# hebbarashwin/neural_polar_decoder

Hardware: AMD Instinct MI355X
Metric: codewords/sec Polar(64,32) SC + CRISP-GRU decode, 1/2/4/8 GPU; BER match (higher is better)
Workload: dtype fp16x3 GRU (hi+lo fp16 MFMA operands, fp32 accumulate/gates); fp32 SC

## Files before the change

neural_polar_decoder_amd/csrc/npd_gru.hip:

```cpp
#include <stdlib.h>
#include <string.h>

#include <new>
#include <type_traits>
#include <vector>

#include "npd_common.hpp"
#include "npd_gru_common.hpp"

namespace npd {
namespace gru {

template <int F, int L, int WPB = NPD_GRU_WPB, int HDT = 0>
__global__ __launch_bounds__(64 * WPB) void gru_decode_kernel(const Args a) {
    constexpr bool FOLD = true, BINIT = true;
    using G = Geo<F, L>;
    constexpr int TT = G::TT, HT = G::HT, KG = G::KG;
    extern __shared__ __attribute__((aligned(16))) f4 smem4[];
    const float* smem = reinterpret_cast<const float*>(smem4);
    {
        const f4* src = reinterpret_cast<const f4*>(a.img);
        for (int i = threadIdx.x; i < G::TOTAL / 4; i += blockDim.x) smem4[i] = src[i];
        __syncthreads();
    }
    const int lane = threadIdx.x & 63;
    const int wave = threadIdx.x >> 6;
    const int half = lane >> 5;
    const int col = lane & 31;
    const int N = a.N;
    const int64_t ntiles = (a.B + 31) / 32;
    const f16v zero = {0.f, 0.f, 0.f, 0.f, 0.f, 0.f, 0.f, 0.f, 0.f, 0.f, 0.f, 0.f, 0.f, 0.f, 0.f, 0.f};
    auto cvec = [&](int off) -> f16v {
        const f4* p = reinterpret_cast<const f4*>(smem + off + half * 16);
        const f4 x0 = p[0], x1 = p[1], x2 = p[2], x3 = p[3];
        return f16v{x0[0], x0[1], x0[2], x0[3], x1[0], x1[1], x1[2], x1[3],
                    x2[0], x2[1], x2[2], x2[3], x3[0], x3[1], x3[2], x3[3]};
    };

    for (int64_t tile = (int64_t)blockIdx.x * WPB + wave; tile < ntiles; tile += (int64_t)gridDim.x * WPB) {
        const int64_t cw = tile * 32 + col;
        const bool valid = cw < a.B;
        const int64_t cwc = valid ? cw : a.B - 1;

        f16v P[TT];
#pragma unroll
        for (int t = 0; t < TT; ++t) P[t] = zero;
        if (a.y) {
            const f4* yr = reinterpret_cast<const f4*>(a.y + cwc * N + half * (N / 2));
            const int ng = N / 8;
            for (int s4 = 0; s4 < ng; ++s4) {
                const f4 yv = yr[s4];
#pragma unroll
                for (int t = 0; t < TT; ++t) {
                    const f4 w = a.wy[(t * ng + s4) * 64 + lane];
                    P[t] = mfma(w.x, yv.x, P[t]);
                    P[t] = mfma(w.y, yv.y, P[t]);
                    P[t] = mfma(w.z, yv.z, P[t]);
// ... 494 lines not shown
    const int64_t tiles = (a.B + 31) / 32;
    const int64_t wgs = (tiles + NPD_GRU_WPB - 1) / NPD_GRU_WPB;
    hipLaunchKernelGGL(kern, dim3(grid_for(wgs, 1, device_cu_count())), dim3(64 * NPD_GRU_WPB), lds, s, a);
    return launch_check("lstm_decode_kernel launch");
}

typedef __bf16 bf8 __attribute__((ext_vector_type(8)));
typedef _Float16 hf8 __attribute__((ext_vector_type(8)));

template <int SPLIT>
struct SplitT {
    static constexpr bool kLo = SPLIT >= 3;
    static constexpr bool kF16 = SPLIT >= 4;
    static constexpr bool kFold = SPLIT == 5;
    using V = std::conditional_t<kF16, hf8, bf8>;
    using E = std::conditional_t<kF16, _Float16, __bf16>;
    static constexpr float kIn = SPLIT == 4 ? 256.0f : 1.0f;
    static constexpr float kAcc = SPLIT == 4 ? 1.0f / 65536.0f : 1.0f;
    static constexpr float kC1 = kFold ? 1.0f : -1.44269504088896340736f * kAcc;
    static constexpr float kC2 = kFold ? 1.0f : -2.88539008177792681472f * kAcc;
};

template <int F, int L, int SPLIT>
struct GeoB {
    static constexpr int TT = 3 * F / 32, HT = F / 32, KB = F / 16;
    static constexpr int NG = (L == 2) ? 3 : 1;
    static constexpr int IMG = NG * TT * KB * 64 * 4;
    static constexpr int NS = SPLIT >= 3 ? 2 : 1;
    static constexpr int OFF_X = NS * IMG;
    static constexpr int OFF_IN = OFF_X + NG * TT * 64;
    static constexpr int OFF_WL = OFF_IN + HT * 64;
    static constexpr int TOTAL = OFF_WL + 2 * HT * 16;
};

struct ArgsB {
    const float* img;
    const f4* wy;
    const float* y;
    const float* h0;
    const float* gt;
    float* decoded;
    float* logits;
    int64_t B;
    int N;
    int rev;
    int onehot;
    float b_lin;
    int64_t wy_lo;
    uint32_t info[kMaxWords];
    const float* msg;
    unsigned long long* counters;
    int K;
    int nseg;
    uint32_t slotw[kMaxN / 4];
};

__device__ __forceinline__ f16v mfma16(const bf8& a, const bf8& b, const f16v& c) {
    return __builtin_amdgcn_mfma_f32_32x32x16_bf16(a, b, c, 0, 0, 0);
}
__device__ __forceinline__ f16v mfma16(const hf8& a, const hf8& b, const f16v& c) {
    return __builtin_amdgcn_mfma_f32_32x32x16_f16(a, b, c, 0, 0, 0);
}


template <int SPLIT>
__device__ __forceinline__ void gru_update_fast(f16v& h, const f16v& ar, const f16v& az, const f16v& ain,
                                                const f16v& ahn) {
    constexpr float c1 = SplitT<SPLIT>::kC1, c2 = SplitT<SPLIT>::kC2;
#pragma unroll
    for (int i = 0; i < 16; ++i) {
        const float r = __builtin_amdgcn_rcpf(1.0f + __builtin_amdgcn_exp2f(c1 * ar[i]));
        const float z = __builtin_amdgcn_rcpf(1.0f + __builtin_amdgcn_exp2f(c1 * az[i]));
        const float x = ain[i] + ahn[i] * r;
        const float nn = fmaf(2.0f, __builtin_amdgcn_rcpf(1.0f + __builtin_amdgcn_exp2f(c2 * x)), -1.0f);
        h[i] = (h[i] - nn) * z + nn;
    }
}

template <int HT, int SPLIT>
__device__ __forceinline__ void to_frags(const f16v (&h)[HT], typename SplitT<SPLIT>::V (&hi)[2 * HT],
                                         typename SplitT<SPLIT>::V (&lo)[2 * HT]) {
    using S = SplitT<SPLIT>;
#pragma unroll
    for (int t = 0; t < HT; ++t)
#pragma unroll
        for (int s = 0; s < 2; ++s)
#pragma unroll
            for (int j = 0; j < 8; ++j) {
                const float v = h[t][8 * s + j] * S::kIn;
                const typename S::E b = (typename S::E)v;
                hi[2 * t + s][j] = b;
                if (S::kLo) lo[2 * t + s][j] = (typename S::E)(v - (float)b);
            }
}

template <int TT, int KB, int NT, int SPLIT, int IMG>
__device__ __forceinline__ void gemm_bf(const f4* __restrict__ smem4, int g, int t0, int lane, f16v (&acc)[NT],
                                        const typename SplitT<SPLIT>::V (&hi)[KB],
                                        const typename SplitT<SPLIT>::V (&lo)[KB]) {
    using V = typename SplitT<SPLIT>::V;
#pragma unroll
    for (int q = 0; q < KB; ++q) {
        V ah[NT], al[NT];
#pragma unroll
        for (int t = 0; t < NT; ++t) {
            const f4 v = smem4[((g * TT + t0 + t) * KB + q) * 64 + lane];
            ah[t] = __builtin_bit_cast(V, v);
// ... 212 lines not shown
                        const size_t e = ((((size_t)(g * TT + t) * KB + q) * 64 + l) * 8 + j);
                        u16[e] = hi;
                        if (SPLIT >= 3) u16[(size_t)GB::IMG * 2 + e] = lo;
                    }
    const float kc = SPLIT == 4 ? 65536.0f : 1.0f;
    for (int i = 0; i < GB::NG * TT * 64; ++i) img[GB::OFF_X + i] = img32[G32::OFF_X + i] * kc;
    for (int i = 0; i < HT * 64; ++i) img[GB::OFF_IN + i] = img32[G32::OFF_IN + i] * kc;
    for (int i = 0; i < 2 * HT * 16; ++i) img[GB::OFF_WL + i] = img32[G32::OFF_WL + i];
    const int nq = N / 16;
    const size_t per = (size_t)TT * nq * 64 * 8;
    wy.assign((per * (SPLIT >= 3 ? 2 : 1) + 1) / 2, 0.0f);
    uint16_t* w16 = reinterpret_cast<uint16_t*>(wy.data());
    for (int t = 0; t < TT; ++t)
        for (int q = 0; q < nq; ++q)
            for (int l = 0; l < 64; ++l)
                for (int j = 0; j < 8; ++j) {
                    const int row = 32 * t + (l & 31);
                    const int k = 16 * q + 8 * (l >> 5) + j;
                    const float v = wih[0][(size_t)row * Din + k];
                    const size_t e = (((size_t)t * nq + q) * 64 + l) * 8 + j;
                    uint16_t hi, lo;
                    split16<SPLIT>(v, hi, lo);
                    w16[e] = hi;
                    if (SPLIT >= 3) w16[per + e] = lo;
                }
    wy_lo = (int64_t)(per / 8);
}

template <int F, int L, int SPLIT>
static int launch_bf(const npd_gru* g, const ArgsB& a, hipStream_t s) {
    using G = GeoB<F, L, SPLIT>;
    auto kern = gru_decode_bf_kernel<F, L, SPLIT>;
    const size_t lds = (size_t)G::TOTAL * 4;
    static bool attr = false;
    if (!attr) {
        NPD_HIP(hipFuncSetAttribute((const void*)kern, hipFuncAttributeMaxDynamicSharedMemorySize, 163840));
        attr = true;
    }
    const int64_t tiles = (a.B + 31) / 32;
    const int64_t wgs = (tiles + NPD_GRU_BF_WPB - 1) / NPD_GRU_BF_WPB;
    const int grid = grid_for(wgs, 1, device_cu_count());
    hipLaunchKernelGGL(kern, dim3(grid), dim3(64 * NPD_GRU_BF_WPB), lds, s, a);
    (void)g;
    return launch_check("gru_decode_bf_kernel launch");
}

struct Geo16 {
    static constexpr int RT = 12, KB = 2, NG = 3;
    static constexpr int IMG4 = NG * RT * KB * 64;
    static constexpr int G_BYTES = RT * KB * 2 * 1024;
    static constexpr int OFF_C = 2 * IMG4 * 4;
    static constexpr int C0L0 = OFF_C, C1L0 = OFF_C + 192, BHN0 = OFF_C + 384, C0L1 = OFF_C + 448,
                         BHN1 = OFF_C + 640, WLIN = OFF_C + 704, TOTAL = OFF_C + 768;
};

__device__ __forceinline__ f4 mfma16s(const hf8& a, const hf8& b, const f4& c) {
    return __builtin_amdgcn_mfma_f32_16x16x32_f16(a, b, c, 0, 0, 0);
}
__device__ __forceinline__ f4 mfma16s(const bf8& a, const bf8& b, const f4& c) {
    return __builtin_amdgcn_mfma_f32_16x16x32_bf16(a, b, c, 0, 0, 0);
}

template <int SPLIT>
__device__ __forceinline__ void split16s(const f4 (&h)[4], typename SplitT<SPLIT>::V (&hi)[2],
                                         typename SplitT<SPLIT>::V (&lo)[2]) {
    using S = SplitT<SPLIT>;
#pragma unroll
    for (int kb = 0; kb < 2; ++kb)
#pragma unroll
        for (int j = 0; j < 8; ++j) {
            const float v = h[2 * kb + (j >> 2)][j & 3] * S::kIn;
            const typename S::E b = (typename S::E)v;
            hi[kb][j] = b;
            if (S::kLo) lo[kb][j] = (typename S::E)(v - (float)b);
        }
}

__device__ __forceinline__ f4 frag16(const f4* __restrict__ smem4, uint32_t wb, int t, int kb, int part) {
    return *reinterpret_cast<const f4*>(reinterpret_cast<const char*>(smem4) + wb +
                                        ((t * Geo16::KB + kb) * 2 + part) * 1024);
}

__device__ __forceinline__ float sum_rows16(float p) {
    const auto r = __builtin_amdgcn_permlane16_swap(__float_as_uint(p), __float_as_uint(p), false, false);
    const float s = __uint_as_float(r[0]) + __uint_as_float(r[1]);
    const auto r2 = __builtin_amdgcn_permlane32_swap(__float_as_uint(s), __float_as_uint(s), false, false);
    return __uint_as_float(r2[0]) + __uint_as_float(r2[1]);
}

__device__ __forceinline__ f4 fma4(float x, const f4& c, const f4& p) {
    return f4{fmaf(x, c[0], p[0]), fmaf(x, c[1], p[1]), fmaf(x, c[2], p[2]), fmaf(x, c[3], p[3])};
}

#define NPD_GRU16_WPB 8
template <int SPLIT>
struct Upd4 {
    f4 er, ez, en, z;
    template <int C>
    __device__ __forceinline__ void step(f4& h, const f4& ar, const f4& az, const f4& ain, const f4& ahn) {
        constexpr float c1 = SplitT<SPLIT>::kC1, c2 = SplitT<SPLIT>::kC2;
        constexpr int i = C / 3, st = C % 3;
        if constexpr (st == 0) {
            er[i] = __builtin_amdgcn_exp2f(c1 * ar[i]);
            ez[i] = __builtin_amdgcn_exp2f(c1 * az[i]);
        } else if constexpr (st == 1) {
            const float r = __builtin_amdgcn_rcpf(1.0f + er[i]);
            z[i] = __builtin_amdgcn_rcpf(1.0f + ez[i]);
            en[i] = __builtin_amdgcn_exp2f(c2 * (ain[i] + ahn[i] * r));
        } else {
            const float nn = fmaf(2.0f, __builtin_amdgcn_rcpf(1.0f + en[i]), -1.0f);
            h[i] = (h[i] - nn) * z[i] + nn;
        }
    }
};

template <int SPLIT>
__device__ __forceinline__ void split_kb(const f4 (&h)[4], int kb, typename SplitT<SPLIT>::V (&hi)[2],
                                         typename SplitT<SPLIT>::V (&lo)[2]) {
    using S = SplitT<SPLIT>;
#pragma unroll
    for (int j = 0; j < 8; ++j) {
        const float v = h[2 * kb + (j >> 2)][j & 3] * S::kIn;
        const typename S::E b = (typename S::E)v;
        hi[kb][j] = b;
        if (S::kLo) lo[kb][j] = (typename S::E)(v - (float)b);
    }
}


template <int SPLIT, int NU>
struct Frag16 {
    typename SplitT<SPLIT>::V h[NU], l[NU];
};
template <int SPLIT, int NU>
__device__ __forceinline__ void load_kb16(const f4* __restrict__ smem4, uint32_t wb, const int (&t)[NU], int kb,
                                          Frag16<SPLIT, NU>& f) {
    using V = typename SplitT<SPLIT>::V;
#pragma unroll
    for (int u = 0; u < NU; ++u) {
        f.h[u] = __builtin_bit_cast(V, frag16(smem4, wb, t[u], kb, 0));
        if (SplitT<SPLIT>::kLo) f.l[u] = __builtin_bit_cast(V, frag16(smem4, wb, t[u], kb, 1));
    }
}

template <int SPLIT, int NU, int C0, int NCH, typename Work>
__device__ __forceinline__ void gemm16i(const f4* __restrict__ smem4, uint32_t wb, const int (&t)[NU],
                                        f4 (&acc)[NU], const typename SplitT<SPLIT>::V (&bh)[2],
                                        const typename SplitT<SPLIT>::V (&bl)[2], Frag16<SPLIT, NU>& cur,
                                        uint32_t wbn, const int (&tn)[NU], Work&& work) {
    constexpr int NT = 2 * NU;
    Frag16<SPLIT, NU> f[2];
    load_kb16<SPLIT, NU>(smem4, wb, t, 1, f[1]);
    asm volatile("" ::: "memory");
    static_for<0, NT>([&](auto trc) {
        constexpr int tr = decltype(trc)::value;
        constexpr int kb = tr / NU, u = tr % NU;
        const Frag16<SPLIT, NU>& F = kb == 0 ? cur : f[kb];
        acc[u] = mfma16s(F.h[u], bh[kb], acc[u]);
        if (SplitT<SPLIT>::kLo) {
            acc[u] = mfma16s(F.h[u], bl[kb], acc[u]);
            acc[u] = mfma16s(F.l[u], bh[kb], acc[u]);
        }
        if constexpr (tr == NU - 1) {
            asm volatile("" ::: "memory");
            load_kb16<SPLIT, NU>(smem4, wbn, tn, 0, cur);
        }
        static_for<C0 + NCH * tr / NT, C0 + NCH * (tr + 1) / NT>([&](auto cc) { work(cc); });
        __builtin_amdgcn_sched_barrier(0);
    });
}

template <int SPLIT>
__global__ __launch_bounds__(64 * NPD_GRU16_WPB) void gru16p_kernel(const ArgsB a) {
    using G = Geo16;
    using S = SplitT<SPLIT>;
    using V = typename S::V;
    using E = typename S::E;
    extern __shared__ __attribute__((aligned(16))) f4 smem4[];
    {
        const f4* src = reinterpret_cast<const f4*>(a.img);
        for (int i = threadIdx.x; i < G::TOTAL / 4; i += blockDim.x) smem4[i] = src[i];
        __syncthreads();
    }
    const int lane = threadIdx.x & 63;
    const int wave = threadIdx.x >> 6;
    const int g4 = lane >> 4;
    const int col = lane & 15;
    const int N = a.N;
    const int nkb = N / 32;
    const int64_t tps = (a.B + 15) / 16;
    const int64_t ntiles = tps * (a.nseg > 1 ? a.nseg : 1);
    const bool count = a.counters != nullptr;
    uint32_t be_w = 0, bl_w = 0;
    uint32_t wbs[3];
#pragma unroll
    for (int g = 0; g < 3; ++g) {
        uint32_t v = g * G::G_BYTES + lane * 16;
        asm volatile("" : "+v"(v));
        wbs[g] = v;
    }
    uint32_t cb = (G::OFF_C + 4 * g4) * 4;
    asm volatile("" : "+v"(cb));
    auto c4 = [&](int off, int t) -> f4 {
        return *reinterpret_cast<const f4*>(reinterpret_cast<const char*>(smem4) + cb + (off - G::OFF_C + 16 * t) * 4);
    };
    const f4 zero = {0.f, 0.f, 0.f, 0.f};
    constexpr int T0[3] = {0, 4, 8};
    auto nowork = [](auto) {};

    for (int64_t tile = (int64_t)blockIdx.x * NPD_GRU16_WPB + wave; tile < ntiles;
         tile += (int64_t)gridDim.x * NPD_GRU16_WPB) {
        const int64_t seg = tile / tps;
        const int64_t cw = (tile - seg * tps) * 16 + col;
        const bool valid = cw < a.B;
        const int64_t cwc = valid ? cw : a.B - 1;
        const int64_t rowoff = (seg * a.B + cw) * N;
        uint32_t mc[4] = {0u, 0u, 0u, 0u};
        if (count) {
            const float* mr = a.msg + cwc * a.K;
#pragma unroll
            for (int w = 0; w < 4; ++w)
                for (int j = 0; j < 16; ++j) {
                    const int sl = 4 * (16 * w + j) + g4;
                    if (sl >= a.K) break;
                    const float v = rintf(mr[sl]);
                    const uint32_t code = v == -1.0f ? 0u : v == 1.0f ? 1u : v == 0.0f ? 2u : 3u;
                    mc[w] |= code << (2 * j);
                }
        }
        uint32_t nerr = 0;
        f4 P[G::RT];
#pragma unroll
        for (int t = 0; t < G::RT; ++t) P[t] = c4(G::C0L0, t);
        if (a.y) {
            const float* yr = a.y + (seg * a.B + cwc) * N;
            for (int kb = 0; kb < nkb; ++kb) {
                const f4 y0 = *reinterpret_cast<const f4*>(yr + 32 * kb + 8 * g4);
                const f4 y1 = *reinterpret_cast<const f4*>(yr + 32 * kb + 8 * g4 + 4);
                V yh, yl;
#pragma unroll
                for (int j = 0; j < 8; ++j) {
                    const float v = (j < 4 ? y0[j] : y1[j - 4]) * S::kIn;
                    yh[j] = (E)v;
                    if (S::kLo) yl[j] = (E)(v - (float)yh[j]);
                }
#pragma unroll
                for (int t = 0; t < G::RT; ++t) {
                    const V wh = __builtin_bit_cast(V, a.wy[(t * nkb + kb) * 64 + lane]);
                    P[t] = mfma16s(wh, yh, P[t]);
                    if (S::kLo) {
                        const V wl = __builtin_bit_cast(V, a.wy[a.wy_lo + (t * nkb + kb) * 64 + lane]);
                        P[t] = mfma16s(wh, yl, P[t]);
                        P[t] = mfma16s(wl, yh, P[t]);
                    }
                }
            }
        }
        f4 h0[4], h1[4];
#pragma unroll
        for (int t = 0; t < 4; ++t) {
            h0[t] = zero;
            h1[t] = zero;
        }
        if (a.h0) {
            const float* hr = a.h0 + (seg * a.B + cwc) * 128;
#pragma unroll
            for (int t = 0; t < 4; ++t)
#pragma unroll
                for (int e = 0; e < 4; ++e) {
                    const int f = 16 * t + 4 * g4 + e;
                    h0[t][e] = hr[2 * f];
                    h1[t][e] = hr[2 * f + 1];
                }
        }
        V fh[2], fl[2], gh[2], gl[2];
        split16s<SPLIT>(h0, fh, fl);
        split16s<SPLIT>(h1, gh, gl);
        float xb = 1.0f;
        f4 a0[3] = {zero, zero, c4(G::BHN0, 0)};
        constexpr int T1[3] = {1, 5, 9};
        Frag16<SPLIT, 3> cur;
        load_kb16<SPLIT, 3>(smem4, wbs[0], T0, 0, cur);
        gemm16i<SPLIT, 3, 0, 0>(smem4, wbs[0], T0, a0, fh, fl, cur, wbs[0], T1, nowork);
        for (int ii = 0; ii < N; ++ii) {
            const int jj = a.rev ? N - 1 - ii : ii;
            Upd4<SPLIT> u;
            const int sl = count ? (int)((a.slotw[jj >> 2] >> (8 * (jj & 3))) & 255u) : 255;
            f4 ap[3] = {a0[0] + fma4(xb, c4(G::C1L0, 0), P[0]), a0[1] + fma4(xb, c4(G::C1L0, 4), P[4]), a0[2]};
            f4 ainp = fma4(xb, c4(G::C1L0, 8), P[8]);
            static_for<1, 4>([&](auto htc) {
                constexpr int ht = decltype(htc)::value;
                const int T[3] = {ht, 4 + ht, 8 + ht};
                f4 acc[3] = {fma4(xb, c4(G::C1L0, ht), P[ht]), fma4(xb, c4(G::C1L0, 4 + ht), P[4 + ht]),
                             c4(G::BHN0, ht)};
                constexpr int TN[3] = {ht < 3 ? ht + 1 : 0, ht < 3 ? 5 + ht : 4, ht < 3 ? 9 + ht : 8};
                gemm16i<SPLIT, 3, 0, 12>(smem4, wbs[0], T, acc, fh, fl, cur, wbs[ht < 3 ? 0 : 2], TN, [&](auto cc) {
                    u.template step<decltype(cc)::value>(h0[ht - 1], ap[0], ap[1], ainp, ap[2]);
                });
                ainp = fma4(xb, c4(G::C1L0, 8 + ht), P[8 + ht]);
#pragma unroll
                for (int k = 0; k < 3; ++k) ap[k] = acc[k];
            });
            f4 b[3] = {c4(G::C0L1, 0), c4(G::C0L1, 4), c4(G::BHN1, 0)};
            gemm16i<SPLIT, 3, 0, 14>(smem4, wbs[2], T0, b, gh, gl, cur, wbs[1], T0, [&](auto cc) {
                constexpr int c = decltype(cc)::value;
                if constexpr (c < 12) u.template step<c>(h0[3], ap[0], ap[1], ainp, ap[2]);
                else split_kb<SPLIT>(h0, c - 12, fh, fl);
            });
            f4 bi[3] = {b[0], b[1], c4(G::C0L1, 8)};
            gemm16i<SPLIT, 3, 0, 0>(smem4, wbs[1], T0, bi, fh, fl, cur, wbs[2], T1, nowork);
            f4 q[4] = {bi[0], bi[1], bi[2], b[2]};
            float part = 0.0f;
            static_for<1, 4>([&](auto htc) {
                constexpr int ht = decltype(htc)::value;
                const int T[3] = {ht, 4 + ht, 8 + ht};
                f4 bb[3] = {c4(G::C0L1, ht), c4(G::C0L1, 4 + ht), c4(G::BHN1, ht)};
                auto work = [&](auto cc) {
                    constexpr int c = decltype(cc)::value;
                    if constexpr (c < 12) {
                        u.template step<c>(h1[ht - 1], q[0], q[1], q[2], q[3]);
                    } else {
                        const f4 wl = c4(G::WLIN, ht - 1);
#pragma unroll
                        for (int i = 0; i < 4; ++i) part = fmaf(wl[i], h1[ht - 1][i], part);
                    }
                };
                gemm16i<SPLIT, 3, 0, 7>(smem4, wbs[2], T, bb, gh, gl, cur, wbs[1], T, work);
                f4 bbi[3] = {bb[0], bb[1], c4(G::C0L1, 8 + ht)};
                constexpr int TN[3] = {ht < 3 ? ht + 1 : 0, ht < 3 ? 5 + ht : 4, ht < 3 ? 9 + ht : 8};
                gemm16i<SPLIT, 3, 7, 6>(smem4, wbs[1], T, bbi, fh, fl, cur, wbs[ht < 3 ? 2 : 0], TN, work);
                q[0] = bbi[0];
                q[1] = bbi[1];
                q[2] = bbi[2];
                q[3] = bb[2];
            });
            a0[0] = zero;
            a0[1] = zero;
            a0[2] = c4(G::BHN0, 0);
            gemm16i<SPLIT, 3, 0, 15>(smem4, wbs[0], T0, a0, fh, fl, cur, wbs[0], T1, [&](auto cc) {
                constexpr int c = decltype(cc)::value;
                if constexpr (c < 12) {
                    u.template step<c>(h1[3], q[0], q[1], q[2], q[3]);
                } else if constexpr (c == 12) {
                    const f4 wl = c4(G::WLIN, 3);
#pragma unroll
                    for (int i = 0; i < 4; ++i) part = fmaf(wl[i], h1[3][i], part);
                    const float out = sum_rows16(part) + a.b_lin;
                    const bool info = (a.info[jj >> 5] >> (jj & 31)) & 1u;
                    float d;
                    if (info) d = out > 0.0f ? 1.0f : (out < 0.0f ? -1.0f : 0.0f);
                    else d = a.gt ? a.gt[(seg * a.B + cwc) * N + jj] : 1.0f;
                    if (g4 == 0 && valid) {
                        if (a.decoded) a.decoded[rowoff + jj] = d;
                        if (a.logits) a.logits[rowoff + ii] = out;
                    }
                    if (sl != 255) {
                        const int q = sl >> 2, w = q >> 4;
                        const uint32_t mw = w == 0 ? mc[0] : w == 1 ? mc[1] : w == 2 ? mc[2] : mc[3];
                        const uint32_t dc = d > 0.0f ? 1u : (d < 0.0f ? 0u : 2u);
                        nerr += (g4 == (sl & 3) && ((mw >> (2 * (q & 15))) & 3u) != dc) ? 1u : 0u;
                    }
                    const float sd = d > 0.0f ? 1.0f : (d < 0.0f ? -1.0f : 0.0f);
                    xb = a.onehot ? (sd > 0.0f ? 1.0f : 0.0f) : sd;
                } else {
                    split_kb<SPLIT>(h1, c - 13, gh, gl);
                }
            });
        }
        if (count) {
            nerr += __shfl_xor(nerr, 16, 64);
            nerr += __shfl_xor(nerr, 32, 64);
            const bool mine = g4 == 0 && valid;
            bl_w += (uint32_t)__builtin_popcountll(__ballot(mine && nerr != 0u));
            uint32_t e = mine ? nerr : 0u;
#pragma unroll
            for (int o = 1; o < 16; o <<= 1) e += __shfl_xor(e, o, 64);
            be_w += (uint32_t)__builtin_amdgcn_readfirstlane(e);
            const int64_t nt = tile + (int64_t)gridDim.x * NPD_GRU16_WPB;
            if (nt >= ntiles || nt / tps != seg) {
                if (lane == 0 && (be_w | bl_w)) {
                    atomicAdd(a.counters + 2 * seg, (unsigned long long)be_w);
                    atomicAdd(a.counters + 2 * seg + 1, (unsigned long long)bl_w);
                }
                be_w = bl_w = 0;
            }
        }
    }
}

template <int SPLIT>
static void build_image16(const float* W, int N, int onehot, std::vector<float>& img, std::vector<float>& wy,
                          int64_t& wy_lo) {
    using G = Geo16;
    constexpr int F = 64, L = 2;
    const int Din = N + (onehot ? 2 : 1);
    const float* p = W;
    const float* wih[2];
    const float* whh[2];
    const float* bih[2];
    const float* bhh[2];
    for (int l = 0; l < L; ++l) {
        const int din = l == 0 ? Din : F;
        wih[l] = p; p += (size_t)3 * F * din;
        whh[l] = p; p += (size_t)3 * F * F;
        bih[l] = p; p += 3 * F;
        bhh[l] = p; p += 3 * F;
    }
    const float* wlin = p;
    img.assign(G::TOTAL, 0.0f);
    const float* mats[3] = {whh[0], wih[1], whh[1]};
    auto fold = [&](int row) { return SPLIT == 5 ? (row < 2 * F ? -1.44269504088896340736f : -2.88539008177792681472f) : 1.0f; };
    uint16_t* u16 = reinterpret_cast<uint16_t*>(img.data());
    for (int g = 0; g < G::NG; ++g)
        for (int t = 0; t < G::RT; ++t)
            for (int kb = 0; kb < G::KB; ++kb)
                for (int l = 0; l < 64; ++l)
                    for (int j = 0; j < 8; ++j) {
                        const int row = 16 * t + (l & 15);
                        const int hid = 16 * (2 * kb + (j >> 2)) + 4 * (l >> 4) + (j & 3);
                        uint16_t hi, lo;
                        split16<SPLIT>(fold(row) * mats[g][(size_t)row * F + hid], hi, lo);
                        const size_t e = (((((size_t)(g * G::RT + t) * G::KB + kb) * 2) * 64 + l) * 8 + j);
                        u16[e] = hi;
                        if (SPLIT >= 3) u16[e + 64 * 8] = lo;
                    }
    const float kc = SPLIT == 4 ? 65536.0f : 1.0f;
    auto col = [&](int row, int k) { return wih[0][(size_t)row * Din + k]; };
    for (int row = 0; row < 3 * F; ++row) {
        const bool rz = row < 2 * F;
        const float c0x = onehot ? col(row, N) : 0.0f;
        const float c1x = onehot ? col(row, N + 1) - col(row, N) : col(row, N);
        img[G::C0L0 + row] = fold(row) * (kc * (rz ? bih[0][row] + bhh[0][row] + c0x : bih[0][row] + c0x));
        img[G::C1L0 + row] = fold(row) * (kc * c1x);
        img[G::C0L1 + row] = fold(row) * (kc * (rz ? bih[1][row] + bhh[1][row] : bih[1][row]));
    }
    for (int j = 0; j < F; ++j) {
        img[G::BHN0 + j] = fold(2 * F + j) * (kc * bhh[0][2 * F + j]);
        img[G::BHN1 + j] = fold(2 * F + j) * (kc * bhh[1][2 * F + j]);
        img[G::WLIN + j] = wlin[j];
    }
    const int nkb = N / 32;
    const size_t per = (size_t)G::RT * nkb * 64 * 8;
    wy.assign((per * (SPLIT >= 3 ? 2 : 1) + 1) / 2, 0.0f);
    uint16_t* w16 = reinterpret_cast<uint16_t*>(wy.data());
    for (int t = 0; t < G::RT; ++t)
        for (int kb = 0; kb < nkb; ++kb)
            for (int l = 0; l < 64; ++l)
                for (int j = 0; j < 8; ++j) {
                    const int row = 16 * t + (l & 15);
                    const int k = 32 * kb + 8 * (l >> 4) + j;
                    uint16_t hi, lo;
                    split16<SPLIT>(fold(row) * col(row, k), hi, lo);
                    const size_t e = (((size_t)t * nkb + kb) * 64 + l) * 8 + j;
                    w16[e] = hi;
                    if (SPLIT >= 3) w16[per + e] = lo;
                }
    wy_lo = (int64_t)(per / 8);
}

template <int SPLIT>
static int launch16(const ArgsB& a, hipStream_t s) {
    auto kern = gru16p_kernel<SPLIT>;
    static bool attr = false;
    if (!attr) {
        NPD_HIP(hipFuncSetAttribute((const void*)kern, hipFuncAttributeMaxDynamicSharedMemorySize, 163840));
        attr = true;
    }
    const int64_t tiles = (a.B + 15) / 16 * (a.nseg > 1 ? a.nseg : 1);
    const int64_t wgs = (tiles + NPD_GRU16_WPB - 1) / NPD_GRU16_WPB;
    const int grid = grid_for(wgs, 1, device_cu_count());
    hipLaunchKernelGGL(kern, dim3(grid), dim3(64 * NPD_GRU16_WPB), (size_t)Geo16::TOTAL * 4, s, a);
    return launch_check("gru16p_kernel launch");
}

template <int F>
struct WideGeo {
    static constexpr int HT = F / 32;
    static constexpr int NW = HT < 8 ? HT : 8;
    static constexpr int HPW = HT / NW;
};

int wide_lds_bytes(int N, int F, int L) {
    const int nw = (F / 32) < 8 ? F / 32 : 8;
    return (L * F * 32 + N * 32 + nw * 32) * 4;
}

template <int HPW, int D0, int D1, int D2>
__device__ __forceinline__ void wide_chain(const f4* __restrict__ W, int kg, int HT, int jt0,
                                           const f4* __restrict__ Bs, int lane, f16v (&acc)[4][HPW]) {
    constexpr int D[3] = {D0, D1, D2};
    f4 wc[3][HPW];
#pragma unroll
    for (int k = 0; k < 3; ++k)
#pragma unroll
        for (int j = 0; j < HPW; ++j) wc[k][j] = W[((size_t)(k * HT + jt0 + j) * kg + 0) * 64 + lane];
    for (int q = 0; q < kg; ++q) {
        f4 wn[3][HPW];
        if (q + 1 < kg) {
#pragma unroll
            for (int k = 0; k < 3; ++k)
#pragma unroll
                for (int j = 0; j < HPW; ++j) wn[k][j] = W[((size_t)(k * HT + jt0 + j) * kg + q + 1) * 64 + lane];
        }
        const f4 b = Bs[q * 64 + lane];
        asm volatile("" ::: "memory");
#pragma unroll
        for (int e = 0; e < 4; ++e)
#pragma unroll
            for (int k = 0; k < 3; ++k)
#pragma unroll
                for (int j = 0; j < HPW; ++j) acc[D[k]][j] = mfma(wc[k][j][e], b[e], acc[D[k]][j]);
        if (q + 1 < kg) {
#pragma unroll
            for (int k = 0; k < 3; ++k)
#pragma unroll
                for (int j = 0; j < HPW; ++j) wc[k][j] = wn[k][j];
        }
    }
}

template <int HPW>
__device__ __forceinline__ void wide_update(f4* __restrict__ Hs, int jt, int lane, f16v& hv, const f16v& ar,
                                            const f16v& az, const f16v& ain, const f16v& ahn) {
#pragma unroll
    for (int q = 0; q < 4; ++q) {
// ... 601 lines not shown
        b.wy = reinterpret_cast<const gru::f4*>(g->wy);
        b.y = y; b.h0 = h0; b.gt = gt; b.decoded = decoded; b.logits = logits; b.B = B; b.N = g->N;
        b.rev = a.rev; b.onehot = a.onehot; b.b_lin = g->b_lin; b.wy_lo = g->wy_lo;
        b.nseg = 1;
        for (int w = 0; w < kMaxWords; ++w) b.info[w] = a.info[w];
        if (g->img16) {
            b.img = g->img16;
            b.wy = reinterpret_cast<const gru::f4*>(g->wy16);
            b.wy_lo = g->wy16_lo;
            return g->split16 == 3 ? gru::launch16<3>(b, s) : g->split16 == 5 ? gru::launch16<5>(b, s)
                                   : gru::launch16<1>(b, s);
        }
#define NPD_LBF(FF, LL)                                                                                   \
        return g->precision == 1   ? gru::launch_bf<FF, LL, 3>(g, b, s)                                     \
               : g->precision == 3 ? gru::launch_bf<FF, LL, 4>(g, b, s)                                     \
                                   : gru::launch_bf<FF, LL, 1>(g, b, s)
        if (g->F == 64 && g->layers == 2) NPD_LBF(64, 2);
        if (g->F == 64) NPD_LBF(64, 1);
        if (g->layers == 2) NPD_LBF(32, 2);
        NPD_LBF(32, 1);
#undef NPD_LBF
    }
    if (g->F > 64) {
        if (g->F == 512) return g->layers == 2 ? gru::launch_wide<512, 2>(a, g->N, s) : gru::launch_wide<512, 1>(a, g->N, s);
        if (g->F == 256) return g->layers == 2 ? gru::launch_wide<256, 2>(a, g->N, s) : gru::launch_wide<256, 1>(a, g->N, s);
        return g->layers == 2 ? gru::launch_wide<128, 2>(a, g->N, s) : gru::launch_wide<128, 1>(a, g->N, s);
    }
    if (g->hd != nullptr) {
#define NPD_LHD(FF, LL) \
        return g->hd_tiles == 1 ? gru::launch<FF, LL, 1>(a, s) : g->hd_tiles == 2 ? gru::launch<FF, LL, 2>(a, s) \
                                                                                   : gru::launch<FF, LL, 4>(a, s)
        if (g->F == 64 && g->layers == 2) NPD_LHD(64, 2);
        if (g->F == 64) NPD_LHD(64, 1);
        if (g->layers == 2) NPD_LHD(32, 2);
        NPD_LHD(32, 1);
#undef NPD_LHD
    }
    if (g->F == 64 && g->layers == 2) return gru::launch<64, 2>(a, s);
    if (g->F == 64) return gru::launch<64, 1>(a, s);
    if (g->layers == 2) return gru::launch<32, 2>(a, s);
    return gru::launch<32, 1>(a, s);
}

extern "C" int npd_gru_decode_count_sweep(const npd_gru* g, int n_seg, const float* y, const uint8_t* is_info,
                                          int reverse, const float* msg, int K, const int32_t* cols, float* decoded,
                                          int64_t B, unsigned long long* counters, void* stream) {
    NPD_ARG(g != nullptr, "npd_gru_decode_count_sweep: gru is NULL");
    NPD_ARG(B >= 0 && n_seg >= 0 && K >= 0, "npd_gru_decode_count_sweep: negative size");
    if (B == 0 || n_seg == 0) return NPD_OK;
    NPD_ARG(y != nullptr && is_info != nullptr && counters != nullptr && (K == 0 || (msg != nullptr && cols != nullptr)),
            "npd_gru_decode_count_sweep: null pointer");
    NPD_ARG(((uintptr_t)y & 15) == 0, "npd_gru_decode_count_sweep: y must be 16-byte aligned");
    NPD_ARG(K <= g->N, "npd_gru_decode_count_sweep: K > N");
    uint8_t slot[kMaxN];
    memset(slot, 255, sizeof(slot));
    for (int k = 0; k < K; ++k) {
        NPD_ARG(cols[k] >= 0 && cols[k] < g->N, "npd_gru_decode_count_sweep: column out of range");
        NPD_ARG(slot[cols[k]] == 255, "npd_gru_decode_count_sweep: repeated column");
        slot[cols[k]] = (uint8_t)k;
    }
    hipStream_t s = (hipStream_t)stream;
    if (g->img16 == nullptr || g->cell != 0) {
        NPD_ARG(decoded != nullptr, "npd_gru_decode_count_sweep: handles other than the 16-codeword split kernel (F = 64, "
                                    "2 layers, N % 32 == 0, precision != 0) need decoded (n_seg, B, N)");
        const int64_t rows = B * g->N;
        for (int sg = 0; sg < n_seg; ++sg) {
            int rc = npd_gru_decode_ex(g, y + sg * rows, nullptr, is_info, reverse, nullptr, decoded + sg * rows, nullptr,
                                       B, stream);
            if (rc == NPD_OK && K > 0)
                rc = npd_count_errors_cols(msg, decoded + sg * rows, B, K, g->N, cols, counters + 2 * sg, stream);
            if (rc != NPD_OK) return rc;
        }
        return NPD_OK;
    }
    gru::ArgsB b{};
    b.img = g->img16;
    b.wy = reinterpret_cast<const gru::f4*>(g->wy16);
    b.wy_lo = g->wy16_lo;
    b.y = y; b.h0 = nullptr; b.gt = nullptr; b.decoded = decoded; b.logits = nullptr; b.B = B; b.N = g->N;
    b.rev = reverse ? 1 : 0; b.onehot = g->onehot; b.b_lin = g->b_lin;
    for (int w = 0; w < kMaxWords; ++w) b.info[w] = 0;
    for (int i = 0; i < g->N; ++i)
        if (is_info[i]) b.info[i >> 5] |= 1u << (i & 31);
    b.msg = msg; b.counters = counters; b.K = K; b.nseg = n_seg;
    memcpy(b.slotw, slot, sizeof(slot));
    return g->split16 == 3 ? gru::launch16<3>(b, s) : g->split16 == 5 ? gru::launch16<5>(b, s) : gru::launch16<1>(b, s);
}

extern "C" int npd_gru_decode(const npd_gru* g, const float* y, const uint8_t* is_info, int reverse, const float* gt,
                              float* decoded, float* logits, int64_t B, void* stream) {
    if (B > 0 && y == nullptr) return fail(NPD_EINVAL, "npd_gru_decode: null pointer");
    return npd_gru_decode_ex(g, y, nullptr, is_info, reverse, gt, decoded, logits, B, stream);
}

namespace npd {
namespace gru {
constexpr int MK = 16;

__device__ __forceinline__ float mlp_act(float x, int act) {
    switch (act) {
        case 1: return x > 0.0f ? x : 0.0f;
        case 2: return 1.0507009873554805f * (x > 0.0f ? x : 1.6732632423543772f * expm1f(x));
        case 3: return x > 0.0f ? x : expm1f(x);
        case 4: return tanhf(x);
        case 5: return 1.0f / (1.0f + expf(-x));
        default: return x;
    }
}

__global__ __launch_bounds__(256) void mlp_layer_kernel(const float* __restrict__ x, const float* __restrict__ W,
                                                        const float* __restrict__ bias, float* __restrict__ out,
                                                        int64_t B, int K, int Nout, int act) {
    __shared__ float xs[64][MK + 1];
    __shared__ float ws[64][MK + 1];
    const int tid = threadIdx.x;
    const int ty = tid >> 4, tx = tid & 15;
    const int64_t m0 = (int64_t)blockIdx.y * 64;
    const int j0 = blockIdx.x * 64;
    float acc[4][4] = {};
    for (int k0 = 0; k0 < K; k0 += MK) {
        for (int e = tid; e < 64 * MK; e += 256) {
            const int r = e / MK, k = e % MK;
            const int64_t m = m0 + r;
            const int j = j0 + r;
            xs[r][k] = (m < B && k0 + k < K) ? x[m * K + k0 + k] : 0.0f;
            ws[r][k] = (j < Nout && k0 + k < K) ? W[(int64_t)j * K + k0 + k] : 0.0f;
        }
        __syncthreads();
#pragma unroll
        for (int k = 0; k < MK; ++k)
#pragma unroll
            for (int i = 0; i < 4; ++i)
#pragma unroll
                for (int c = 0; c < 4; ++c) acc[i][c] = fmaf(xs[ty + 16 * i][k], ws[tx + 16 * c][k], acc[i][c]);
        __syncthreads();
    }
#pragma unroll
    for (int i = 0; i < 4; ++i) {
// ... 24 lines not shown
```

Baseline: 78.42 million.

## Specialize count-only GRU16 kernel, move slot/info table to LDS, rebalance MFMA work interleave

Adds an IO template flag so the count-only sweep path skips the decoded/logits/gt writes and the float decision logic, replacing them with branchless pos/neg bit logic. Per-position slot and info bits are packed into an LDS table and read once per step via readfirstlane, instead of extracting them from kernel arguments. The interleaving of GRU gate-update work across MFMA triples is rebalanced with explicit cut maps: the layer-1 split work moves into earlier GEMMs and a few constant loads are hoisted or prefetched. The cost is a slightly larger LDS footprint, a second kernel instantiation, and scheduling changes that may shift register pressure.

```diff
diff --git a/neural_polar_decoder_amd/csrc/npd_gru.hip b/neural_polar_decoder_amd/csrc/npd_gru.hip
--- a/neural_polar_decoder_amd/csrc/npd_gru.hip
+++ b/neural_polar_decoder_amd/csrc/npd_gru.hip
@@ -3,6 +3,7 @@
 
 #include <new>
 #include <type_traits>
+#include <utility>
 #include <vector>
 
 #include "npd_common.hpp"
@@ -603,7 +604,8 @@
     unsigned long long* counters;
     int K;
     int nseg;
-    uint32_t slotw[kMaxN / 4];
+    static constexpr uint16_t kNoSlot = 0xFFFF;
+    uint16_t slot[kMaxN];
 };
 
 __device__ __forceinline__ f16v mfma16(const bf8& a, const bf8& b, const f16v& c) {
@@ -922,6 +924,7 @@
     static constexpr int OFF_C = 2 * IMG4 * 4;
     static constexpr int C0L0 = OFF_C, C1L0 = OFF_C + 192, BHN0 = OFF_C + 384, C0L1 = OFF_C + 448,
                          BHN1 = OFF_C + 640, WLIN = OFF_C + 704, TOTAL = OFF_C + 768;
+    static constexpr int STAB = TOTAL, LDS_FLOATS = TOTAL + kMaxN;
 };
 
 __device__ __forceinline__ f4 mfma16s(const hf8& a, const hf8& b, const f4& c) {
@@ -996,6 +999,18 @@
         if (S::kLo) lo[kb][j] = (typename S::E)(v - (float)b);
     }
 }
+template <int SPLIT>
+__device__ __forceinline__ void split_half(const f4 (&h)[4], int kb, int half, typename SplitT<SPLIT>::V (&hi)[2],
+                                           typename SplitT<SPLIT>::V (&lo)[2]) {
+    using S = SplitT<SPLIT>;
+#pragma unroll
+    for (int j = 4 * half; j < 4 * half + 4; ++j) {
+        const float v = h[2 * kb + half][j & 3] * S::kIn;
+        const typename S::E b = (typename S::E)v;
+        hi[kb][j] = b;
+        if (S::kLo) lo[kb][j] = (typename S::E)(v - (float)b);
+    }
+}
 
 
 template <int SPLIT, int NU>
@@ -1013,12 +1028,30 @@
     }
 }
 
-template <int SPLIT, int NU, int C0, int NCH, typename Work>
+template <int... B>
+struct Cuts {
+    static constexpr int n = sizeof...(B);
+    static constexpr int at(int i) {
+        constexpr int v[] = {B...};
+        return v[i];
+    }
+};
+template <int NT, int C0, int NCH, typename = std::make_integer_sequence<int, NT + 1>>
+struct EvenT;
+template <int NT, int C0, int NCH, int... I>
+struct EvenT<NT, C0, NCH, std::integer_sequence<int, I...>> {
+    using type = Cuts<(C0 + NCH * I / NT)...>;
+};
+template <int NT, int C0, int NCH>
+using Even = typename EvenT<NT, C0, NCH>::type;
+
+template <int SPLIT, int NU, typename MAP, typename Work>
 __device__ __forceinline__ void gemm16i(const f4* __restrict__ smem4, uint32_t wb, const int (&t)[NU],
                                         f4 (&acc)[NU], const typename SplitT<SPLIT>::V (&bh)[2],
                                         const typename SplitT<SPLIT>::V (&bl)[2], Frag16<SPLIT, NU>& cur,
                                         uint32_t wbn, const int (&tn)[NU], Work&& work) {
     constexpr int NT = 2 * NU;
+    static_assert(MAP::n == NT + 1, "one chunk bound per triple, and the end");
     Frag16<SPLIT, NU> f[2];
     load_kb16<SPLIT, NU>(smem4, wb, t, 1, f[1]);
     asm volatile("" ::: "memory");
@@ -1035,21 +1068,26 @@
             asm volatile("" ::: "memory");
             load_kb16<SPLIT, NU>(smem4, wbn, tn, 0, cur);
         }
-        static_for<C0 + NCH * tr / NT, C0 + NCH * (tr + 1) / NT>([&](auto cc) { work(cc); });
+        static_for<MAP::at(tr), MAP::at(tr + 1)>([&](auto cc) { work(cc); });
         __builtin_amdgcn_sched_barrier(0);
     });
 }
 
-template <int SPLIT>
+template <int SPLIT, bool IO>
 __global__ __launch_bounds__(64 * NPD_GRU16_WPB) void gru16p_kernel(const ArgsB a) {
     using G = Geo16;
     using S = SplitT<SPLIT>;
     using V = typename S::V;
     using E = typename S::E;
     extern __shared__ __attribute__((aligned(16))) f4 smem4[];
+    uint32_t* const stab = reinterpret_cast<uint32_t*>(smem4) + G::STAB;
     {
         const f4* src = reinterpret_cast<const f4*>(a.img);
         for (int i = threadIdx.x; i < G::TOTAL / 4; i += blockDim.x) smem4[i] = src[i];
+        for (int j = threadIdx.x; j < kMaxN; j += blockDim.x) {
+            const uint32_t sl = a.counters != nullptr && j < a.N ? a.slot[j] : ArgsB::kNoSlot;
+            stab[j] = sl | (((a.info[j >> 5] >> (j & 31)) & 1u) << 16);
+        }
         __syncthreads();
     }
     const int lane = threadIdx.x & 63;
@@ -1060,7 +1098,7 @@
     const int nkb = N / 32;
     const int64_t tps = (a.B + 15) / 16;
     const int64_t ntiles = tps * (a.nseg > 1 ? a.nseg : 1);
-    const bool count = a.counters != nullptr;
+    const bool count = !IO || a.counters != nullptr;
     uint32_t be_w = 0, bl_w = 0;
     uint32_t wbs[3];
 #pragma unroll
@@ -1077,6 +1115,7 @@
     const f4 zero = {0.f, 0.f, 0.f, 0.f};
     constexpr int T0[3] = {0, 4, 8};
     auto nowork = [](auto) {};
+    const float xneg = a.onehot ? 0.0f : -1.0f;
 
     for (int64_t tile = (int64_t)blockIdx.x * NPD_GRU16_WPB + wave; tile < ntiles;
          tile += (int64_t)gridDim.x * NPD_GRU16_WPB) {
@@ -1085,13 +1124,15 @@
         const bool valid = cw < a.B;
         const int64_t cwc = valid ? cw : a.B - 1;
         const int64_t rowoff = (seg * a.B + cw) * N;
+        int g4t = g4, lanet = lane;
+        asm volatile("" : "+v"(g4t), "+v"(lanet));
         uint32_t mc[4] = {0u, 0u, 0u, 0u};
         if (count) {
             const float* mr = a.msg + cwc * a.K;
 #pragma unroll
             for (int w = 0; w < 4; ++w)
                 for (int j = 0; j < 16; ++j) {
-                    const int sl = 4 * (16 * w + j) + g4;
+                    const int sl = 4 * (16 * w + j) + g4t;
                     if (sl >= a.K) break;
                     const float v = rintf(mr[sl]);
                     const uint32_t code = v == -1.0f ? 0u : v == 1.0f ? 1u : v == 0.0f ? 2u : 3u;
@@ -1105,8 +1146,8 @@
         if (a.y) {
             const float* yr = a.y + (seg * a.B + cwc) * N;
             for (int kb = 0; kb < nkb; ++kb) {
-                const f4 y0 = *reinterpret_cast<const f4*>(yr + 32 * kb + 8 * g4);
-                const f4 y1 = *reinterpret_cast<const f4*>(yr + 32 * kb + 8 * g4 + 4);
+                const f4 y0 = *reinterpret_cast<const f4*>(yr + 32 * kb + 8 * g4t);
+                const f4 y1 = *reinterpret_cast<const f4*>(yr + 32 * kb + 8 * g4t + 4);
                 V yh, yl;
 #pragma unroll
                 for (int j = 0; j < 8; ++j) {
@@ -1116,10 +1157,10 @@
                 }
 #pragma unroll
                 for (int t = 0; t < G::RT; ++t) {
-                    const V wh = __builtin_bit_cast(V, a.wy[(t * nkb + kb) * 64 + lane]);
+                    const V wh = __builtin_bit_cast(V, a.wy[(t * nkb + kb) * 64 + lanet]);
                     P[t] = mfma16s(wh, yh, P[t]);
                     if (S::kLo) {
-                        const V wl = __builtin_bit_cast(V, a.wy[a.wy_lo + (t * nkb + kb) * 64 + lane]);
+                        const V wl = __builtin_bit_cast(V, a.wy[a.wy_lo + (t * nkb + kb) * 64 + lanet]);
                         P[t] = mfma16s(wh, yl, P[t]);
                         P[t] = mfma16s(wl, yh, P[t]);
                     }
@@ -1138,7 +1179,7 @@
             for (int t = 0; t < 4; ++t)
 #pragma unroll
                 for (int e = 0; e < 4; ++e) {
-                    const int f = 16 * t + 4 * g4 + e;
+                    const int f = 16 * t + 4 * g4t + e;
                     h0[t][e] = hr[2 * f];
                     h1[t][e] = hr[2 * f + 1];
                 }
@@ -1151,34 +1192,43 @@
         constexpr int T1[3] = {1, 5, 9};
         Frag16<SPLIT, 3> cur;
         load_kb16<SPLIT, 3>(smem4, wbs[0], T0, 0, cur);
-        gemm16i<SPLIT, 3, 0, 0>(smem4, wbs[0], T0, a0, fh, fl, cur, wbs[0], T1, nowork);
+        gemm16i<SPLIT, 3, Even<6, 0, 0>>(smem4, wbs[0], T0, a0, fh, fl, cur, wbs[0], T1, nowork);
+        f4 cx[3] = {c4(G::C1L0, 1), c4(G::C1L0, 5), c4(G::BHN0, 1)};
         for (int ii = 0; ii < N; ++ii) {
             const int jj = a.rev ? N - 1 - ii : ii;
             Upd4<SPLIT> u;
-            const int sl = count ? (int)((a.slotw[jj >> 2] >> (8 * (jj & 3))) & 255u) : 255;
             f4 ap[3] = {a0[0] + fma4(xb, c4(G::C1L0, 0), P[0]), a0[1] + fma4(xb, c4(G::C1L0, 4), P[4]), a0[2]};
             f4 ainp = fma4(xb, c4(G::C1L0, 8), P[8]);
             static_for<1, 4>([&](auto htc) {
                 constexpr int ht = decltype(htc)::value;
                 const int T[3] = {ht, 4 + ht, 8 + ht};
-                f4 acc[3] = {fma4(xb, c4(G::C1L0, ht), P[ht]), fma4(xb, c4(G::C1L0, 4 + ht), P[4 + ht]),
-                             c4(G::BHN0, ht)};
+                f4 acc[3] = {fma4(xb, ht == 1 ? cx[0] : c4(G::C1L0, ht), P[ht]),
+                             fma4(xb, ht == 1 ? cx[1] : c4(G::C1L0, 4 + ht), P[4 + ht]), ht == 1 ? cx[2] : c4(G::BHN0, ht)};
                 constexpr int TN[3] = {ht < 3 ? ht + 1 : 0, ht < 3 ? 5 + ht : 4, ht < 3 ? 9 + ht : 8};
-                gemm16i<SPLIT, 3, 0, 12>(smem4, wbs[0], T, acc, fh, fl, cur, wbs[ht < 3 ? 0 : 2], TN, [&](auto cc) {
-                    u.template step<decltype(cc)::value>(h0[ht - 1], ap[0], ap[1], ainp, ap[2]);
-                });
+                if constexpr (ht == 1) {
+                    gemm16i<SPLIT, 3, Even<6, 0, 12>>(smem4, wbs[0], T, acc, fh, fl, cur, wbs[0], TN, [&](auto cc) {
+                        u.template step<decltype(cc)::value>(h0[0], ap[0], ap[1], ainp, ap[2]);
+                    });
+                } else {
+                    gemm16i<SPLIT, 3, Cuts<0, 2, 4, 7, 9, 12, 14>>(smem4, wbs[0], T, acc, fh, fl, cur,
+                                                                   wbs[ht < 3 ? 0 : 2], TN, [&](auto cc) {
+                        constexpr int c = decltype(cc)::value;
+                        if constexpr (c == 5 || c == 10) split_half<SPLIT>(h1, ht - 2, c == 10, gh, gl);
+                        else u.template step<(c < 5 ? c : c < 10 ? c - 1 : c - 2)>(h0[ht - 1], ap[0], ap[1], ainp, ap[2]);
+                    });
+                }
                 ainp = fma4(xb, c4(G::C1L0, 8 + ht), P[8 + ht]);
 #pragma unroll
                 for (int k = 0; k < 3; ++k) ap[k] = acc[k];
             });
             f4 b[3] = {c4(G::C0L1, 0), c4(G::C0L1, 4), c4(G::BHN1, 0)};
-            gemm16i<SPLIT, 3, 0, 14>(smem4, wbs[2], T0, b, gh, gl, cur, wbs[1], T0, [&](auto cc) {
+            gemm16i<SPLIT, 3, Even<6, 0, 14>>(smem4, wbs[2], T0, b, gh, gl, cur, wbs[1], T0, [&](auto cc) {
                 constexpr int c = decltype(cc)::value;
                 if constexpr (c < 12) u.template step<c>(h0[3], ap[0], ap[1], ainp, ap[2]);
                 else split_kb<SPLIT>(h0, c - 12, fh, fl);
             });
             f4 bi[3] = {b[0], b[1], c4(G::C0L1, 8)};
-            gemm16i<SPLIT, 3, 0, 0>(smem4, wbs[1], T0, bi, fh, fl, cur, wbs[2], T1, nowork);
+            gemm16i<SPLIT, 3, Even<6, 0, 0>>(smem4, wbs[1], T0, bi, fh, fl, cur, wbs[2], T1, nowork);
             f4 q[4] = {bi[0], bi[1], bi[2], b[2]};
             float part = 0.0f;
             static_for<1, 4>([&](auto htc) {
@@ -1195,10 +1245,10 @@
                         for (int i = 0; i < 4; ++i) part = fmaf(wl[i], h1[ht - 1][i], part);
                     }
                 };
-                gemm16i<SPLIT, 3, 0, 7>(smem4, wbs[2], T, bb, gh, gl, cur, wbs[1], T, work);
+                gemm16i<SPLIT, 3, Even<6, 0, 7>>(smem4, wbs[2], T, bb, gh, gl, cur, wbs[1], T, work);
                 f4 bbi[3] = {bb[0], bb[1], c4(G::C0L1, 8 + ht)};
                 constexpr int TN[3] = {ht < 3 ? ht + 1 : 0, ht < 3 ? 5 + ht : 4, ht < 3 ? 9 + ht : 8};
-                gemm16i<SPLIT, 3, 7, 6>(smem4, wbs[1], T, bbi, fh, fl, cur, wbs[ht < 3 ? 2 : 0], TN, work);
+                gemm16i<SPLIT, 3, Even<6, 7, 6>>(smem4, wbs[1], T, bbi, fh, fl, cur, wbs[ht < 3 ? 2 : 0], TN, work);
                 q[0] = bbi[0];
                 q[1] = bbi[1];
                 q[2] = bbi[2];
@@ -1207,33 +1257,47 @@
             a0[0] = zero;
             a0[1] = zero;
             a0[2] = c4(G::BHN0, 0);
-            gemm16i<SPLIT, 3, 0, 15>(smem4, wbs[0], T0, a0, fh, fl, cur, wbs[0], T1, [&](auto cc) {
+            f4 wl3;
+            uint32_t sw;
+            gemm16i<SPLIT, 3, Cuts<0, 3, 6, 9, 12, 13, 14>>(smem4, wbs[0], T0, a0, fh, fl, cur, wbs[0], T1, [&](auto cc) {
                 constexpr int c = decltype(cc)::value;
-                if constexpr (c < 12) {
+                if constexpr (c == 13) {
+                    cx[0] = c4(G::C1L0, 1);
+                    cx[1] = c4(G::C1L0, 5);
+                    cx[2] = c4(G::BHN0, 1);
+                } else if constexpr (c < 12) {
+                    if constexpr (c == 0) sw = stab[jj];
+                    if constexpr (c == 9) wl3 = c4(G::WLIN, 3);
                     u.template step<c>(h1[3], q[0], q[1], q[2], q[3]);
-                } else if constexpr (c == 12) {
-                    const f4 wl = c4(G::WLIN, 3);
-#pragma unroll
-                    for (int i = 0; i < 4; ++i) part = fmaf(wl[i], h1[3][i], part);
+                } else {
+#pragma unroll
+                    for (int i = 0; i < 4; ++i) part = fmaf(wl3[i], h1[3][i], part);
                     const float out = sum_rows16(part) + a.b_lin;
-                    const bool info = (a.info[jj >> 5] >> (jj & 31)) & 1u;
-                    float d;
-                    if (info) d = out > 0.0f ? 1.0f : (out < 0.0f ? -1.0f : 0.0f);
-                    else d = a.gt ? a.gt[(seg * a.B + cwc) * N + jj] : 1.0f;
-                    if (g4 == 0 && valid) {
-                        if (a.decoded) a.decoded[rowoff + jj] = d;
-                        if (a.logits) a.logits[rowoff + ii] = out;
+                    const uint32_t sws = (uint32_t)__builtin_amdgcn_readfirstlane((int)sw);
+                    const bool info = (sws >> 16) & 1u;
+                    bool pos, neg;
+                    if constexpr (IO) {
+                        float d;
+                        if (info) d = out > 0.0f ? 1.0f : (out < 0.0f ? -1.0f : 0.0f);
+                        else d = a.gt ? a.gt[(seg * a.B + cwc) * N + jj] : 1.0f;
+                        if (g4 == 0 && valid) {
+                            if (a.decoded) a.decoded[rowoff + jj] = d;
+                            if (a.logits) a.logits[rowoff + ii] = out;
+                        }
+                        pos = d > 0.0f;
+                        neg = d < 0.0f;
+                    } else {
+                        pos = !info | (out > 0.0f);
+                        neg = info & (out < 0.0f);
                     }
-                    if (sl != 255) {
-                        const int q = sl >> 2, w = q >> 4;
-                        const uint32_t mw = w == 0 ? mc[0] : w == 1 ? mc[1] : w == 2 ? mc[2] : mc[3];
-                        const uint32_t dc = d > 0.0f ? 1u : (d < 0.0f ? 0u : 2u);
-                        nerr += (g4 == (sl & 3) && ((mw >> (2 * (q & 15))) & 3u) != dc) ? 1u : 0u;
-                    }
-                    const float sd = d > 0.0f ? 1.0f : (d < 0.0f ? -1.0f : 0.0f);
-                    xb = a.onehot ? (sd > 0.0f ? 1.0f : 0.0f) : sd;
-                } else {
-                    split_kb<SPLIT>(h1, c - 13, gh, gl);
+                    const uint32_t sl = sws & 0xFFFFu, q = sl >> 2, w = q >> 4;
+                    const uint32_t m01 = (w & 1u) ? mc[1] : mc[0], m23 = (w & 1u) ? mc[3] : mc[2];
+                    const uint32_t mw = (w & 2u) ? m23 : m01;
+                    const uint32_t dc = pos ? 1u : (neg ? 0u : 2u);
+                    const bool err = (sl != ArgsB::kNoSlot) & ((uint32_t)g4 == (sl & 3u)) &
+                                     (((mw >> (2 * (q & 15u))) & 3u) != dc);
+                    nerr += err ? 1u : 0u;
+                    xb = pos ? 1.0f : (neg ? xneg : 0.0f);
                 }
             });
         }
@@ -1328,9 +1392,9 @@
     wy_lo = (int64_t)(per / 8);
 }
 
-template <int SPLIT>
-static int launch16(const ArgsB& a, hipStream_t s) {
-    auto kern = gru16p_kernel<SPLIT>;
+template <int SPLIT, bool IO>
+static int launch16v(const ArgsB& a, hipStream_t s) {
+    auto kern = gru16p_kernel<SPLIT, IO>;
     static bool attr = false;
     if (!attr) {
         NPD_HIP(hipFuncSetAttribute((const void*)kern, hipFuncAttributeMaxDynamicSharedMemorySize, 163840));
@@ -1339,8 +1403,14 @@
     const int64_t tiles = (a.B + 15) / 16 * (a.nseg > 1 ? a.nseg : 1);
     const int64_t wgs = (tiles + NPD_GRU16_WPB - 1) / NPD_GRU16_WPB;
     const int grid = grid_for(wgs, 1, device_cu_count());
-    hipLaunchKernelGGL(kern, dim3(grid), dim3(64 * NPD_GRU16_WPB), (size_t)Geo16::TOTAL * 4, s, a);
+    hipLaunchKernelGGL(kern, dim3(grid), dim3(64 * NPD_GRU16_WPB), (size_t)Geo16::LDS_FLOATS * 4, s, a);
     return launch_check("gru16p_kernel launch");
+}
+
+template <int SPLIT>
+static int launch16(const ArgsB& a, hipStream_t s) {
+    const bool io = a.counters == nullptr || a.decoded != nullptr || a.logits != nullptr || a.gt != nullptr;
+    return io ? launch16v<SPLIT, true>(a, s) : launch16v<SPLIT, false>(a, s);
 }
 
 template <int F>
@@ -2048,12 +2118,12 @@
             "npd_gru_decode_count_sweep: null pointer");
     NPD_ARG(((uintptr_t)y & 15) == 0, "npd_gru_decode_count_sweep: y must be 16-byte aligned");
     NPD_ARG(K <= g->N, "npd_gru_decode_count_sweep: K > N");
-    uint8_t slot[kMaxN];
-    memset(slot, 255, sizeof(slot));
+    uint16_t slot[kMaxN];
+    for (int i = 0; i < kMaxN; ++i) slot[i] = gru::ArgsB::kNoSlot;
     for (int k = 0; k < K; ++k) {
         NPD_ARG(cols[k] >= 0 && cols[k] < g->N, "npd_gru_decode_count_sweep: column out of range");
-        NPD_ARG(slot[cols[k]] == 255, "npd_gru_decode_count_sweep: repeated column");
-        slot[cols[k]] = (uint8_t)k;
+        NPD_ARG(slot[cols[k]] == gru::ArgsB::kNoSlot, "npd_gru_decode_count_sweep: repeated column");
+        slot[cols[k]] = (uint16_t)k;
     }
     hipStream_t s = (hipStream_t)stream;
     if (g->img16 == nullptr || g->cell != 0) {
@@ -2079,7 +2149,7 @@
     for (int i = 0; i < g->N; ++i)
         if (is_info[i]) b.info[i >> 5] |= 1u << (i & 31);
     b.msg = msg; b.counters = counters; b.K = K; b.nseg = n_seg;
-    memcpy(b.slotw, slot, sizeof(slot));
+    memcpy(b.slot, slot, sizeof(slot));
     return g->split16 == 3 ? gru::launch16<3>(b, s) : g->split16 == 5 ? gru::launch16<5>(b, s) : gru::launch16<1>(b, s);
 }
 
```

Measured after the change: 79.09 million (median of 6 runs). No clear change (+0.8%).
